# Kaz-K/medical-image-editing

Measured on AMD Instinct MI355X. Metric: images/sec (train step, 256x256 2D slices), higher is better.
Workload: dtype f32

## Files before the change

include/vqwnet_hip.h:

```cpp
#ifndef VQWNET_HIP_H
#define VQWNET_HIP_H
#include <stddef.h>
#include <stdint.h>

#define VQW_ABI_VERSION 9

#ifdef __cplusplus
extern "C" {
#endif

const char* vqw_last_error(void);
int vqw_abi_version(void);
int vqw_set_conv_backend(int mode);
int vqw_profile_begin(void);
int vqw_profile_end(double* out);
int vqw_profile_families(unsigned mask);

int vqw_conv2d_fwd(const float* src0, int C0, int up0, const float* src1, int C1,
                   const float* w_ohwi, const float* bias, float* y,
                   int N, int H, int W, int Cout, int ksize, int dil, int relu, void* stream);
int vqw_pack_dgrad_weights(const float* w_ohwi, float* wt, int Cout, int Cin, int ksize, void* stream);
int vqw_conv2d_fwd_stats_parts(int C0, int C1, int up0, int N, int H, int W, int Cout, int ksize, int dil);
int vqw_conv2d_fwd_stats(const float* src0, int C0, int up0, const float* src1, int C1,
                         const float* w_ohwi, const float* bias, float* y, float* part,
// ... 23 lines not shown
                              void* stream);
int vqw_conv3x3_up2_wgrad_supported(int Cin, int Cout, int N, int h, int w);
size_t vqw_conv3x3_up2_wgrad_ws_bytes(int Cin, int Cout, int N, int h, int w);
int vqw_conv3x3_up2_wgrad(const float* x_low, const float* dy, float* dw_ohwi, float* dbias, void* ws, size_t ws_bytes,
                          int N, int h, int w, int Cin, int Cout, int accumulate, void* stream);
int vqw_conv3x3_wino_supported(int Cin, int Cout, int N, int H, int W);
size_t vqw_conv3x3_wino_ws_bytes(int Cin, int Cout);
int vqw_conv3x3_wino_prepare(const float* w_ohwi, void* ws, size_t ws_bytes, int Cin, int Cout, void* stream);
int vqw_conv3x3_wino_prepare_dgrad(const float* w_ohwi, void* ws, size_t ws_bytes, int Cin, int Cout, void* stream);
int vqw_conv3x3_wino_fwd(const float* x, const void* ws, const float* bias, float* y, int N, int H, int W, int Cin, int Cout,
                         int relu, void* stream);
int vqw_conv3x3_wino_masked_supported(int Cin, int Cout, int N, int H, int W);
int vqw_conv3x3_wino_fwd_masked(const float* x, const void* ws, const float* mask, float* y, int N, int H, int W, int Cin,
                                int Cout, void* stream);
int vqw_conv3x3_wino_fwd_acc(const float* x, const void* ws, float* y, int N, int H, int W, int Cin, int Cout, void* stream);
int vqw_conv3x3_wino_dil2_supported(int Cin, int Cout, int N, int H, int W);
int vqw_conv3x3_wino_dil2_stats_parts(int Cin, int Cout, int N, int H, int W);
int vqw_conv3x3_wino_dil2_fwd(const float* x, const void* ws, const float* bias, float* y, float* part, int accumulate,
                              int N, int H, int W, int Cin, int Cout, int relu, void* stream);
int vqw_conv3x3_wino_split_supported(int Cin, int Cout, int split, int pool0, int N, int H, int W);
int vqw_conv3x3_wino_fwd_split(const float* x, const void* ws, const float* bias, float* y0, float* y1, int N, int H, int W,
                               int Cin, int Cout, int split, int pool0, int relu, void* stream);
int vqw_conv3x3_wino_split_padded_supported(int Cin, int Cout, int split, int c1, int pool0, int N, int H, int W);
int vqw_conv3x3_wino_fwd_split_padded(const float* x, const void* ws, const float* bias, float* y0, float* y1, int N, int H, int W,
                                      int Cin, int Cout, int split, int c1, int pool0, int relu, void* stream);
int vqw_conv3x3_wino_fwd_inbwd_parts(int Cin, int Cout, int N, int H, int W);
int vqw_conv3x3_wino_fwd_inbwd(const float* x, const void* ws, const float* norm_x, const float* norm_mean_rstd, int norm_relu,
                               float* y, float* part, int N, int H, int W, int Cin, int Cout, void* stream);
int vqw_conv3x3_wino_fwd_stats_parts(int Cin, int Cout, int N, int H, int W);
int vqw_conv3x3_wino_fwd_stats(const float* x, const void* ws, const float* bias, float* y, float* part, int N, int H, int W,
// ... 35 lines not shown
int vqw_spade_fwd(const float* x, const float* mean_rstd , const float* gamma,
                  const float* beta, int gb_stride, float* y, long P, int C, int relu, void* stream);
int vqw_spade_fwd_res(const float* x, const float* mean_rstd, const float* gamma, const float* beta, int gb_stride,
                      const float* res, float* y, long P, int C, int relu, void* stream);
int vqw_spade_fwd_res_norm_supported(long HW, int C);
int vqw_spade_fwd_res_norm(const float* x, const float* mean_rstd, const float* gamma, const float* beta, int gb_stride,
                           const float* res_raw, const float* res_mean_rstd, int res_relu, float* y, int N, long HW, int C,
                           int relu, void* stream);
int vqw_spade_bwd_reduce(const float* x, const float* mean_rstd, const float* gamma, const float* beta,
                         const float* gy, float* dgamma, float* dbeta, int gb_stride,
                         double* sums , void* ws, size_t ws_bytes, int N, int HW, int C,
                         int relu, void* stream);
int vqw_spade_bwd_apply(const float* x, const float* mean_rstd, const float* gamma, const float* beta,
                        int gb_stride, const float* gy, const double* sums, double count, float* gx,
                        long P, int C, int relu, int training, void* stream);

int vqw_add(const float* a, const float* b, float* y, long n, int relu, void* stream);
int vqw_relu_bwd(const float* y, const float* gy, float* gx, long n, void* stream);
int vqw_maxpool2_fwd(const float* x, float* y, int N, int H, int W, int C, void* stream);
int vqw_maxpool2_bwd(const float* x, const float* gy, const float* g_skip , float* gx,
                     int N, int H, int W, int C, void* stream);
int vqw_res_tail_fwd(const float* a, const float* b, float* out, float* pooled, int N, int H, int W, int C, void* stream);
int vqw_res_tail_norm_fwd(const float* x2, const float* mr2, const float* xid, const float* mrid, float* out, float* pooled,
                          int N, int H, int W, int C, void* stream);
int vqw_res_tail_bwd(const float* out, const float* g_pooled , const float* g_out , float* gx,
                     int N, int H, int W, int C, void* stream);
int vqw_tanh_fwd(const float* x, float* y, long n, void* stream);
int vqw_tanh_bwd(const float* y, const float* gy, float* gx, long n, void* stream);
int vqw_affine(const float* x, float* y, float scale, float shift, long n, void* stream);
int vqw_mse_fwd(const float* a, const float* b, float* loss, void* ws, size_t ws_bytes, long n, void* stream);
// ... 308 lines not shown
```

medical-image-editing_amd/csrc/conv.hip:

```cpp
#include "common.h"
#include <stdlib.h>
#include "conv_common.h"
#include "prof.h"
#include "../../include/vqwnet_hip.h"

static int g_conv_backend = 0;

#define PROF_MAX 32768
static bool g_prof_on = false;
static int g_prof_n = 0;
static hipEvent_t* g_prof_ev = nullptr;
static double g_prof_flops[PROF_MAX];
static double g_prof_bytes[PROF_MAX];
static int g_prof_family[PROF_MAX];

extern "C" int vqw_profile_begin(void) {
    if (!g_prof_ev) {
        g_prof_ev = (hipEvent_t*)malloc(sizeof(hipEvent_t) * 2 * PROF_MAX);
        for (int i = 0; i < 2 * PROF_MAX; ++i)
            if (hipEventCreate(&g_prof_ev[i]) != hipSuccess) { vqw_set_error("vqw_profile_begin: hipEventCreate failed"); return VQW_ERR_HIP; }
    }
    g_prof_n = 0;
    g_prof_on = true;
    return VQW_OK;
// ... 344 lines not shown
extern "C" int vqw_conv3x3_wino_fwd_masked(const float* x, const void* ws, const float* mask, float* y, int N, int H, int W, int Cin,
                                           int Cout, void* stream) {
    VQW_CHECK(x && ws && mask && y && N > 0 && H > 0 && W > 0, "vqw_conv3x3_wino_fwd_masked: bad arguments");
    VQW_CHECK(vqw_conv3x3_wino_masked_supported(Cin, Cout, N, H, W), "vqw_conv3x3_wino_fwd_masked: unsupported shape (query vqw_conv3x3_wino_masked_supported)");
    const double px = (double)N * H * W;
    ProfScope ps(4, 2.0 * px * 4.0 * Cout * Cin, (hipStream_t)stream, 4.0 * (px * Cin + 2.0 * px * Cout + 16.0 * Cout * Cin));
    return conv_wino_fwd(x, (const float*)ws, nullptr, y, N, H, W, Cin, Cout, 0, (hipStream_t)stream, nullptr, mask);
}
extern "C" int vqw_conv3x3_wino_fwd_acc(const float* x, const void* ws, float* y, int N, int H, int W, int Cin, int Cout, void* stream) {
    VQW_CHECK(x && ws && y && N > 0 && H > 0 && W > 0, "vqw_conv3x3_wino_fwd_acc: bad arguments");
    VQW_CHECK(vqw_conv3x3_wino_masked_supported(Cin, Cout, N, H, W), "vqw_conv3x3_wino_fwd_acc: unsupported shape (query vqw_conv3x3_wino_masked_supported)");
    const double px = (double)N * H * W;
    ProfScope ps(4, 2.0 * px * 4.0 * Cout * Cin, (hipStream_t)stream, 4.0 * (px * Cin + 2.0 * px * Cout + 16.0 * Cout * Cin));
    return conv_wino_fwd(x, (const float*)ws, nullptr, y, N, H, W, Cin, Cout, 0, (hipStream_t)stream, nullptr, nullptr, 1);
}
extern "C" int vqw_conv3x3_wino_dil2_supported(int Cin, int Cout, int N, int H, int W) {
    if (g_conv_backend != 0 || N < 1 || H < 2 || W < 2) return 0;
    if (!conv_wino_ok(Cin, Cout, N, H / 2, W / 2) || !conv_wino64_dil2_ok(Cin, Cout, H, W)) return 0;
    return (long)N * H * W * (Cin > Cout ? Cin : Cout) * 4 <= 0xFFFFFFE0L ? 1 : 0;
}
extern "C" int vqw_conv3x3_wino_dil2_stats_parts(int Cin, int Cout, int N, int H, int W) {
    if (!vqw_conv3x3_wino_dil2_supported(Cin, Cout, N, H, W)) return 0;
    return 4 * conv_wino64_stat_tiles(Cin, Cout, H / 2, W / 2);
}
extern "C" int vqw_conv3x3_wino_dil2_fwd(const float* x, const void* ws, const float* bias, float* y, float* part, int accumulate,
                                         int N, int H, int W, int Cin, int Cout, int relu, void* stream) {
    VQW_CHECK(x && ws && y && N > 0 && H > 0 && W > 0, "vqw_conv3x3_wino_dil2_fwd: bad arguments");
    VQW_CHECK(vqw_conv3x3_wino_dil2_supported(Cin, Cout, N, H, W), "vqw_conv3x3_wino_dil2_fwd: unsupported shape (query vqw_conv3x3_wino_dil2_supported)");
    VQW_CHECK(!part || (!relu && !accumulate && vqw_conv3x3_wino_dil2_stats_parts(Cin, Cout, N, H, W) > 0),
              "vqw_conv3x3_wino_dil2_fwd: statistics partials need relu == 0, accumulate == 0 and a served height");
// ... 73 lines not shown
```

medical-image-editing_amd/csrc/conv_common.h:

```cpp
#pragma once
#include "common.h"
#include <cstdlib>

inline int conv_max_blocks() {
    static const int v = [] {
        const char* e = getenv("VQW_CONV_MAX_BLOCKS");
        const int b = e ? atoi(e) : 256;
        return b < 8 ? 8 : (b > 256 ? 256 : b);
    }();
    return v;
}

inline int conv_slab_split(int nsp, int nblk, int max_slabs, int* kt_out) {
    int nsb = conv_max_blocks() / nblk;
    if (nsb > max_slabs) nsb = max_slabs;
    if (nsb > nsp) nsb = nsp;
    if (nsb < 1) nsb = 1;
    const int kt = (nsp + nsb - 1) / nsb;
    if (kt_out) *kt_out = kt;
    return (nsp + kt - 1) / kt;
}
inline int conv_region_runs(int nsp, int ntn, int wg_per_cu) {
    int groups = conv_max_blocks() * wg_per_cu / ntn;
    if (groups < 1) groups = 1;
// ... 77 lines not shown
bool conv_dil_wgrad_ok(const ConvIn& in, int N, int H, int W, int Cout, int ks, int dil);
int conv_dil_wgrad(const ConvIn& in, const float* dy, float* dw, float* ws, int max_slabs, int N, int H, int W, int Cout, int dil,
                   int acc, hipStream_t st);
extern int g_wino_mode;
bool conv_wino_ok(int Cin, int Cout, int N, int H, int W);
size_t conv_wino_ws_floats(int Cin, int Cout);
int conv_wino_prepare(const float* w, float* u, int Cin, int Cout, hipStream_t st, int transposed = 0);
int conv_wino_stat_tiles(int Cin, int Cout, int H, int W);
bool conv_wino64_ok(int Cin, int Cout, int W);
int conv_wino64_stat_tiles(int Cin, int Cout, int H, int W);
bool conv_wino64_split_ok(int Cin, int Cout, int split, int pool0, int N, int H, int W, int c1 = 0);
int conv_wino64_fwd_split(const float* x, const float* u, const float* bias, float* y0, float* y1, int N, int H, int W, int Cin, int Cout,
                          int split, int pool0, int relu, hipStream_t st, int c1 = 0);
int conv_wino64_fwd(const float* x, const float* u, const float* bias, float* y, int N, int H, int W, int Cin, int Cout, int relu,
                    hipStream_t st, float* stats = nullptr, const float* mask = nullptr, int accumulate = 0,
                    const float* in_mr = nullptr, int in_relu = 0, int dil = 1);
bool conv_wino64_dil2_ok(int Cin, int Cout, int H, int W);
int conv_wino_fwd(const float* x, const float* u, const float* bias, float* y, int N, int H, int W, int Cin, int Cout, int relu,
                  hipStream_t st, float* stats = nullptr, const float* mask = nullptr, int accumulate = 0,
                  const float* in_mr = nullptr, int in_relu = 0);
bool conv_wino_wgrad_ok(int Cin, int Cout, int N, int H, int W);
int conv_wino_wgrad_blocks(const ConvIn& in, int Cout, int N, int H, int W, int max_slabs, int* kt_out);
bool conv_wino_blk_wgrad_ok(int C0, int C1, int up0, int Cout, int H, int W);
bool conv_wino_blk_wgrad_dil2_ok(int C0, int Cout, int H, int W);
int conv_wino_blk_wgrad_blocks(int Cin, int Cout, int N, int H, int W, int max_slabs, int* kt_out);
int conv_wino_blk_wgrad(const ConvIn& in, const float* dy, float* ws, float* bpart, int N, int H, int W, int Cin, int Cout, int nsb, int kt,
                        hipStream_t st, int dil = 1);
int conv_wino_wgrad(const ConvIn& in, const float* dy, float* ws, float* bpart, int N, int H, int W, int Cout, int nsb, int kt,
                    hipStream_t st);
bool conv_wino_up_dgrad_ok(int Cin, int Cout, int N, int h, int w);
size_t conv_wino_up_ws_floats(int Cin, int Cout);
// ... 76 lines not shown
```

medical-image-editing_amd/csrc/conv_wino64.hip:

```cpp
#include "common.h"
#include "conv_common.h"
#include "mfma_util.h"
#include "wino_common.h"

extern int g_wino_mode;

namespace {

struct W64Args {
    const float* x;
    const float* u;
    const float* bias;
    float* y;
    int N, H, W, Cin, Cout;
    int tilesY, tilesX, nsp;
    int ntn, nch;
    int kt;
    int relu;
    unsigned nbx, nbu, nby;
    float* stats;
    const float* mask;
    const float* mr;
    int in_relu;
    float* y2;
    int split, pool0;
    int c1;
    unsigned nby2;
    unsigned img_px, rowb_px, rpx, ppx;
    int n_sh, n_m;
};

constexpr int W6_KPH = wino::KPH;
template <int RW, int MBW, int NW = 8> struct W64Geo {
    static_assert(MBW == 1 || (MBW == 2 && RW == 32), "two M blocks per wave: 32-wide regions only");
    static_assert(NW == 8 || (NW == 4 && RW == 32), "four-wave workgroups: 32-wide regions only");
    static constexpr int NMB = NW / 2;
    static constexpr int NBW = 4 / MBW;
    static constexpr int NCO = 16 * NBW;
    static constexpr int TR = RW == 32 ? 2 * MBW * NMB : 16;
    static constexpr int HR = TR + 2, HWV = RW + 2;
    static constexpr int HWS = RW == 32 ? 34 : 24;
    static constexpr int HBUF = HR * HWS * W6_KPH;
    static constexpr int UBUF = 16 * NCO * 8;
    static constexpr int EXF = 2048 * NW;
    static_assert(EXF >= UBUF, "U buffer 1 lives in the exchange area");
    static constexpr size_t LDS_FLOATS = 2 * HBUF + UBUF + EXF + 2 * NMB * NCO * 2;
};
constexpr int W6_LS = 4;
constexpr int W6_ULS = 2;
constexpr int W6_CP = 48;

template <int RW, int MBW, int EPI, int NW = 8>
__global__ void __launch_bounds__(64 * NW, 8 / NW) k_conv_wino64(W64Args a) {
    constexpr bool MASK = EPI >= 1 && EPI <= 3;
    using G = W64Geo<RW, MBW, NW>;
    constexpr int NT = 64 * NW, NMB = G::NMB, NBW = G::NBW, NCO = G::NCO;
    constexpr int HWS = G::HWS, HWV = G::HWV, HBUF = G::HBUF, UBUF = G::UBUF;
    using Halo = wino::HaloStager<NT, G::HR, HWV, HWS, wino::PitchedPix>;
    constexpr int LH = Halo::LH;
    constexpr int LU = 512 * NBW / NT;
    constexpr int HP0 = 1 + LU * W6_ULS;
    static_assert(HP0 + (LH - 1) * W6_LS < W6_CP && W6_CP + LH <= 64, "prefetch slots fit the item");

    extern __shared__ __attribute__((aligned(16))) float smem[];
    float* Hs = smem;
    float* Us = smem + 2 * HBUF;
    float* Ex = Us + UBUF;
    float* Rs = Ex + G::EXF;

    const int tid = threadIdx.x, lane = tid & 63;
    const int wv = __builtin_amdgcn_readfirstlane(tid >> 6);
    const int mb = wv & (NMB - 1), h = wv / NMB;
    const int H = a.H, W = a.W, Cin = a.Cin, Cout = a.Cout;
    const __amdgpu_buffer_rsrc_t rsx = make_rsrc(a.x, a.nbx), rsu = make_rsrc(a.u, a.nbu), rsy = make_rsrc(a.y, a.nby);
    const __amdgpu_buffer_rsrc_t rsm = make_rsrc((EPI == 1 || EPI == 3) ? a.mask : a.y, a.nby);
    const __amdgpu_buffer_rsrc_t rsr = make_rsrc(EPI == 3 ? a.mr : a.y, EPI == 3 ? (unsigned)((size_t)a.N * a.Cout * 8) : a.nby);
    const __amdgpu_buffer_rsrc_t rsy2 = make_rsrc(EPI == 4 ? a.y2 : a.y, EPI == 4 ? a.nby2 : a.nby);

    const int nch = a.nch;
    const wino::RegionRun run = wino::region_run(a.ntn, a.kt, a.nsp);
    const int co_base = run.tile_n * NCO;
    const int my_tiles = run.my_tiles;
    if (my_tiles <= 0) return;

    const int c4 = tid & 1;
    const wino::PitchedPix pixel = {a.img_px, a.rowb_px, a.rpx, a.ppx, a.n_sh, a.n_m};
    Halo hs;
    hs.init(tid, pixel);
    auto region_offsets = [&](int n, int tx, int ty) { hs.region_offsets(n, ty * G::TR - 1, tx * RW - 1, H, W, Cin); };
    const int u_n = (tid >> 1) & (NCO - 1);
    const int u_swz = (u_n >> 3) & 1;
    const int u_c4 = c4 ^ u_swz;
    const unsigned u_voff = (((unsigned)(tid >> 1) / NCO * Cout + co_base + u_n) * 8u + u_c4 * 4) * 4u;
    const unsigned u_jstride = (unsigned)(NT / 2 / NCO) * Cout * 32u;
    const unsigned u_cstride = 16u * Cout * 32u;
    const int u_wave = wv * 256;

    auto issue_h = [&](int j, int chunk) { hs.issue_h(rsx, j, chunk); };
    auto commit_h = [&](int j, float* Hb) { hs.commit_h(j, Hb); };
    auto issue_u = [&](int j, int chunk, float* Ub) {
        wino::buf_ld4_lds(rsu, Ub + u_wave + j * (NT * 4), u_voff, chunk * u_cstride + j * u_jstride);
    };

    int cn, ctx, cty, ch = 0;
    region_start(run.sp0, a.tilesY, a.tilesX, cn, ctx, cty);
    auto advance = [&](int& n, int& tx, int& ty, int& c) {
        const int adv = c + 1 == nch ? 1 : 0;
        c = adv ? 0 : c + 1;
        region_step(adv, a.tilesY, a.tilesX, n, tx, ty);
    };
    int n1 = cn, tx1 = ctx, ty1 = cty, ch1 = 0;
    advance(n1, tx1, ty1, ch1);
    int n2 = n1, tx2 = tx1, ty2 = ty1, ch2 = ch1;
// ... 340 lines not shown
}

static int wino64_shape(int Cin, int Cout, int W) {
    if (Cin % 16 != 0) return 0;
    if (Cout % 64 == 0) return 1;
    return (Cout % 32 == 0 && W % 32 == 0) ? 2 : 0;
}
static int wino64_waves(int shape) { return shape == 2 ? 4 : 8; }
bool conv_wino64_ok(int Cin, int Cout, int W) { return wino64_shape(Cin, Cout, W) != 0; }
int conv_wino64_stat_tiles(int Cin, int Cout, int H, int W) {
    const int shape = wino64_shape(Cin, Cout, W);
    const int rw = W % 32 == 0 ? 32 : 16, tr = rw == 32 ? shape * wino64_waves(shape) : 16;
    return tr > 0 && H % tr == 0 ? (H / tr) * (W / rw) : 0;
}

template <int RW, int MBW, int EPI, int NW = 8>
static int launch_wino64(W64Args& a, hipStream_t st) {
    using G = W64Geo<RW, MBW, NW>;
    constexpr size_t lds = G::LDS_FLOATS * sizeof(float);
    static_assert(lds * (8 / NW) <= 160 * 1024, "buffers do not fit the 160 KB LDS");
    if (int rc = lds_opt_in<k_conv_wino64<RW, MBW, EPI, NW>>((int)lds, "conv_wino64")) return rc;
    a.tilesY = ceil_div(a.H, G::TR); a.tilesX = a.W / RW; a.nsp = a.N * a.tilesY * a.tilesX;
    a.ntn = a.Cout / G::NCO;
    a.kt = conv_region_runs(a.nsp, a.ntn, 8 / NW);
    k_conv_wino64<RW, MBW, EPI, NW><<<ceil_div(a.nsp, a.kt) * a.ntn, 64 * NW, lds, st>>>(a);
    VQW_LAUNCH_CHECK("conv_wino64");
    return VQW_OK;
}

bool conv_wino64_dil2_ok(int Cin, int Cout, int H, int W) {
    return H % 2 == 0 && W % 64 == 0 && wino64_shape(Cin, Cout, W / 2) != 0;
}
int conv_wino64_fwd(const float* x, const float* u, const float* bias, float* y, int N, int H, int W, int Cin, int Cout, int relu,
                    hipStream_t st, float* stats, const float* mask, int accumulate, const float* in_mr, int in_relu, int dil) {
    W64Args a;
    const long P = (long)N * H * W;
    a.img_px = (unsigned)(H * W); a.rowb_px = 0; a.rpx = (unsigned)W; a.ppx = 1; a.n_sh = 0; a.n_m = 0;
    if (dil == 2) {
        a.rowb_px = (unsigned)W; a.rpx = 2u * (unsigned)W; a.ppx = 2; a.n_sh = 2; a.n_m = 1;
        N *= 4; H /= 2; W /= 2;
    }
    a.y2 = nullptr; a.split = 0; a.pool0 = 0; a.c1 = 0; a.nby2 = 0;
    a.x = x; a.u = u; a.bias = bias; a.y = y; a.mask = mask; a.mr = in_mr; a.in_relu = in_relu;
    a.N = N; a.H = H; a.W = W; a.Cin = Cin; a.Cout = Cout;
    a.nch = Cin / 8;
    a.relu = relu;
    a.stats = stats;
    a.nbx = (unsigned)(P * Cin * 4);
    a.nbu = (unsigned)(16L * Cout * Cin * 4);
    a.nby = (unsigned)(P * Cout * 4);
    const int shape = wino64_shape(Cin, Cout, W);
    if (in_mr) {
        if (shape == 2) return launch_wino64<32, 2, 3, 4>(a, st);
        if (W % 32 == 0) return launch_wino64<32, 1, 3>(a, st);
        return launch_wino64<16, 1, 3>(a, st);
    }
    if (mask) {
        if (shape == 2) return launch_wino64<32, 2, 1, 4>(a, st);
        if (W % 32 == 0) return launch_wino64<32, 1, 1>(a, st);
        return launch_wino64<16, 1, 1>(a, st);
    }
    if (accumulate) {
        if (shape == 2) return launch_wino64<32, 2, 2, 4>(a, st);
        if (W % 32 == 0) return launch_wino64<32, 1, 2>(a, st);
        return launch_wino64<16, 1, 2>(a, st);
    }
    if (shape == 2) return launch_wino64<32, 2, 0, 4>(a, st);
    if (W % 32 == 0) return launch_wino64<32, 1, 0>(a, st);
    return launch_wino64<16, 1, 0>(a, st);
}

bool conv_wino64_split_ok(int Cin, int Cout, int split, int pool0, int N, int H, int W, int c1) {
    if (c1 < 0 || c1 % 16 != 0 || split + c1 > Cout) return false;
    if (!conv_wino64_ok(Cin, Cout, W) || g_wino_mode != 0 || split <= 0 || split >= Cout || split % 16 != 0) return false;
    if (pool0 && (H % 2 != 0)) return false;
    return (long)N * H * W * (Cin > Cout ? Cin : Cout) * 4 <= 0xFFFFFFE0L;
}
int conv_wino64_fwd_split(const float* x, const float* u, const float* bias, float* y0, float* y1, int N, int H, int W, int Cin, int Cout,
                          int split, int pool0, int relu, hipStream_t st, int c1) {
    if (c1 <= 0) c1 = Cout - split;
    W64Args a;
    a.img_px = (unsigned)(H * W); a.rowb_px = 0; a.rpx = (unsigned)W; a.ppx = 1; a.n_sh = 0; a.n_m = 0;
    a.x = x; a.u = u; a.bias = bias; a.y = y0; a.y2 = y1; a.mask = nullptr; a.mr = nullptr; a.in_relu = 0;
    a.split = split; a.pool0 = pool0; a.c1 = c1;
    a.N = N; a.H = H; a.W = W; a.Cin = Cin; a.Cout = Cout;
    a.nch = Cin / 8;
    a.relu = relu;
    a.stats = nullptr;
    const long P = (long)N * H * W;
    a.nbx = (unsigned)(P * Cin * 4);
    a.nbu = (unsigned)(16L * Cout * Cin * 4);
    a.nby = (unsigned)((pool0 ? P / 4 : P) * split * 4);
    a.nby2 = (unsigned)(P * c1 * 4);
    const int shape = wino64_shape(Cin, Cout, W);
    if (shape == 2) return launch_wino64<32, 2, 4, 4>(a, st);
    if (W % 32 == 0) return launch_wino64<32, 1, 4>(a, st);
    return launch_wino64<16, 1, 4>(a, st);
}
// ... 357 lines not shown
```

medical-image-editing_amd/csrc/norm.hip:

```cpp
#include <type_traits>
#include "common.h"
#include "prof.h"
#include "../../include/vqwnet_hip.h"

#define PLANE_MAX_SPLITS 64

static inline int plane_splits(int N, int HW) {
    int s = ceil_div(2048, N);
    int cap = imax(1, HW / 256);
    s = imin(imin(s, cap), PLANE_MAX_SPLITS);
    return imax(s, 1);
}

static inline size_t plane_part_bytes(int N, int C) { return (size_t)N * PLANE_MAX_SPLITS * C * 2 * sizeof(double); }
extern "C" size_t vqw_plane_ws_bytes(int N, int C, int HW) {
    (void)HW;
    return plane_part_bytes(N, C) + (size_t)N * C * 2 * sizeof(float);
}

__device__ __forceinline__ float norm_xhat(float x, float mean, float rstd) { return (x - mean) * rstd; }
__device__ __forceinline__ void stats_terms(float v, float& a, float& b) { a = v; b = v * v; }
__device__ __forceinline__ float inorm_bwd_term(float g, float xh, bool relu) { return (relu && !(xh > 0.f)) ? 0.f : g; }
__device__ __forceinline__ float inorm_bwd_out(float gg, float xh, float rstd, float e0, float e1) { return rstd * (gg - e0 - xh * e1); }
__device__ __forceinline__ float spade_out(float xh, float gamma, float beta) { return xh * (1.f + gamma) + beta; }
// ... 770 lines not shown
            }
#pragma unroll
        for (int u = 0; u < 4; ++u) {
            if (p0 + u * R >= P) break;
            float4 o = spade4(v[u], ga[u], be[u], m0, m1, RELU);
            if (RES) { o.x += rr[u].x; o.y += rr[u].y; o.z += rr[u].z; o.w += rr[u].w; }
            y[(p0 + u * R) * C4 + c4] = o;
        }
    }
}

template <int RELU, int TRAIN>
__global__ void __launch_bounds__(256) k_spade_bwd_apply4w(const float4* __restrict__ x, const float* __restrict__ mr,
                                                           const float4* __restrict__ gamma, const float4* __restrict__ beta,
                                                           const float4* __restrict__ gy, const double* __restrict__ sums,
                                                           double inv_count, float4* __restrict__ gx, long P, int C4, int lgC4, int gbs4) {
    WALK4_SETUP;
    const float4 m0 = ((const float4*)(mr + 8 * c4))[0], m1 = ((const float4*)(mr + 8 * c4))[1];
    float s1[4], s2[4];
    spade_bwd_means4(sums, inv_count, c4, TRAIN, s1, s2);
    for (long p0 = (long)blockIdx.x * 2 * R + r; p0 < P; p0 += (long)gridDim.x * 2 * R) {
        float4 v[2], ga4[2], g4[2], be4[2];
#pragma unroll
        for (int u = 0; u < 2; ++u)
            if (p0 + u * R < P) {
                const long p = p0 + u * R;
                v[u] = x[p * C4 + c4]; ga4[u] = gamma[p * gbs4 + c4]; g4[u] = gy[p * C4 + c4];
                be4[u] = RELU ? beta[p * gbs4 + c4] : make_float4(0.f, 0.f, 0.f, 0.f);
            }
#pragma unroll
        for (int u = 0; u < 2; ++u) {
            if (p0 + u * R >= P) break;
            gx[(p0 + u * R) * C4 + c4] = spade_bwd4(v[u], g4[u], ga4[u], be4[u], m0, m1, s1, s2, RELU, TRAIN);
        }
    }
}
static inline int walk_blocks_flat(long P, int C4, int per_step) {
    const int R = 256 / C4;
    long g = (P + (long)per_step * R - 1) / ((long)per_step * R);
    return (int)(g > 2048 ? 2048 : (g < 1 ? 1 : g));
}

// ... 527 lines not shown
    with_flag(relu, [&](auto R) {
        constexpr int RELU = decltype(R)::value;
        if (pick_tier(C, gb_stride, x, gamma, beta, gy, dgamma, dbeta, mean_rstd) != TIER_SCALAR)
            splits = launch_plane_reduce4(FSpadeBwd4<RELU>{(const float4*)x, mean_rstd, (const float4*)gamma, (const float4*)beta, (const float4*)gy,
                                                           (float4*)dgamma, (float4*)dbeta, C / 4, gb_stride / 4}, (double*)ws, N, HW, C, st);
        else splits = launch_plane_reduce(FSpadeBwd<RELU>{x, mean_rstd, gamma, beta, gy, dgamma, dbeta, C, gb_stride}, (double*)ws, N, HW, C, st);
    });
    k_channel_finalize<SplitSums, false><<<C, 256, 0, st>>>(SplitSums{(const double*)ws, N * splits}, sums, C, BnOut{});
    VQW_LAUNCH_CHECK("vqw_spade_bwd_reduce");
    return VQW_OK;
}

template <int RELU, int TRAIN>
__global__ void k_spade_bwd_apply(const float* __restrict__ x, const float* __restrict__ mr, const float* __restrict__ gamma,
                                  const float* __restrict__ beta, const float* __restrict__ gy, const double* __restrict__ sums,
                                  double inv_count, float* __restrict__ gx, long total, int C, int gbs) {
    long stride = (long)gridDim.x * blockDim.x;
    for (long i = (long)blockIdx.x * blockDim.x + threadIdx.x; i < total; i += stride) {
        int c = (int)(i % C);
        long j = (i / C) * gbs + c;
        float r = mr[2 * c + 1];
        float xh = norm_xhat(x[i], mr[2 * c], r);
        float dg, db, dxh;
        spade_bwd_grad(gy[i], xh, gamma[j], RELU ? beta[j] : 0.f, RELU, dg, db, dxh);
        float s1 = TRAIN ? (float)(sums[2 * c] * inv_count) : 0.f;
        float s2 = TRAIN ? (float)(sums[2 * c + 1] * inv_count) : 0.f;
        gx[i] = spade_bwd_out(dxh, xh, r, s1, s2, TRAIN);
    }
}
template <int RELU, int TRAIN>
__global__ void __launch_bounds__(256) k_spade_bwd_apply4(const float4* __restrict__ x, const float* __restrict__ mr,
                                                          const float4* __restrict__ gamma, const float4* __restrict__ beta,
                                                          const float4* __restrict__ gy, const double* __restrict__ sums,
                                                          double inv_count, float4* __restrict__ gx, long total4, int C4, int gbs4) {
    long stride = (long)gridDim.x * blockDim.x;
    for (long i = (long)blockIdx.x * blockDim.x + threadIdx.x; i < total4; i += stride) {
        int c4 = (int)(i % C4);
        long j = (i / C4) * gbs4 + c4;
        const float4* m = (const float4*)(mr + 8 * c4);
        const float4 m0 = m[0], m1 = m[1], v = x[i], ga = gamma[j], g = gy[i];
        const float4 be = RELU ? beta[j] : make_float4(0.f, 0.f, 0.f, 0.f);
        float s1[4], s2[4];
        spade_bwd_means4(sums, inv_count, c4, TRAIN, s1, s2);
        gx[i] = spade_bwd4(v, g, ga, be, m0, m1, s1, s2, RELU, TRAIN);
    }
}
extern "C" int vqw_spade_bwd_apply(const float* x, const float* mean_rstd, const float* gamma, const float* beta, int gb_stride,
                                   const float* gy, const double* sums, double count, float* gx, long P, int C,
                                   int relu, int training, void* stream) {
    VQW_PROF_HBM(stream, 4, (double)P * C);
    VQW_CHECK(x && mean_rstd && gamma && beta && gy && gx && P > 0 && C > 0 && gb_stride >= C, "vqw_spade_bwd_apply: bad arguments");
    VQW_CHECK(!training || (sums && count > 0), "vqw_spade_bwd_apply: training needs sums and count");
    const long total = P * C;
    hipStream_t st = (hipStream_t)stream;
    const double ic = training ? 1.0 / count : 0.0;
    const Tier tier = pick_tier(C, gb_stride, x, gamma, beta, gy, gx, mean_rstd);
    const int C4 = C / 4, s4 = gb_stride / 4;
    const float4 *x4 = (const float4*)x, *ga4 = (const float4*)gamma, *be4 = (const float4*)beta, *gy4 = (const float4*)gy;
    with_flag(relu, [&](auto R) {
        with_flag(training, [&](auto T) {
            constexpr int RELU = decltype(R)::value, TRAIN = decltype(T)::value;
            if (tier == TIER_WALK4)
                k_spade_bwd_apply4w<RELU, TRAIN><<<walk_blocks_flat(P, C4, 2), 256, 0, st>>>(x4, mean_rstd, ga4, be4, gy4, sums, ic, (float4*)gx, P, C4, ilog2_exact(C4), s4);
            else if (tier == TIER_FLAT4)
                k_spade_bwd_apply4<RELU, TRAIN><<<stream_grid(total / 4, 256), 256, 0, st>>>(x4, mean_rstd, ga4, be4, gy4, sums, ic, (float4*)gx, total / 4, C4, s4);
            else k_spade_bwd_apply<RELU, TRAIN><<<stream_grid(total, 256), 256, 0, st>>>(x, mean_rstd, gamma, beta, gy, sums, ic, gx, total, C, gb_stride);
        });
    });
    VQW_LAUNCH_CHECK("vqw_spade_bwd_apply");
    return VQW_OK;
}

__global__ void k_bn_affine_fwd(const float* __restrict__ x, const float* __restrict__ mr, const float* __restrict__ gamma,
                                const float* __restrict__ beta, float* __restrict__ y, long total, int C, float slope) {
    long stride = (long)gridDim.x * blockDim.x;
    for (long i = (long)blockIdx.x * blockDim.x + threadIdx.x; i < total; i += stride) {
        int c = (int)(i % C);
        float v = ((x[i] - mr[2 * c]) * mr[2 * c + 1]) * gamma[c] + beta[c];
        y[i] = v > 0.f ? v : v * slope;
    }
}
extern "C" int vqw_bn_affine_fwd(const float* x, const float* mean_rstd, const float* gamma, const float* beta, float* y, long P,
                                 int C, float slope, void* stream) {
    VQW_CHECK(x && mean_rstd && gamma && beta && y && P > 0 && C > 0, "vqw_bn_affine_fwd: bad arguments");
// ... 70 lines not shown
```

medical-image-editing_amd/hipops/ops.py:

```python
import contextlib
import ctypes
import math
import os

import torch
import torch.distributed as dist

from . import _lib
from .library import Dispatch as _D

CL = torch.channels_last


_dispatch = None


def _L():
    global _dispatch
    if _dispatch is None:
        _dispatch = _D()
    return _dispatch


def _raw(t):
# ... 467 lines not shown
        self._armed_for = None

    def put(self, grad, payload):
        tid = _pass_id()
        if tid >= 0 and self._armed_for != tid:
            self._armed_for = tid
            torch.autograd.Variable._execution_engine.queue_callback(self.clear)
        self.notes[grad.data_ptr()] = (grad._version, tid, payload)

    def take(self, grad):
        ent = self.notes.pop(grad.data_ptr(), None)
        if ent is None or ent[0] != grad._version or ent[1] != _pass_id():
            return None
        return ent[2]

    def clear(self):
        self.notes.clear()
        self._armed_for = None

    def __len__(self):
        return len(self.notes)


UP_PAIR = os.environ.get("VQW_UP_PAIR", "1") != "0"
up_pair_calls = 0
CONV_PAIR = os.environ.get("VQW_CONV_PAIR", "1") != "0"
conv_pair_calls = 0


class _ConvPair(torch.autograd.Function):

    @staticmethod
    def forward(ctx, x, wa, ba, wb, bb, relu, group, up):
        global up_pair_calls, conv_pair_calls
        _dev(x, wa, ba, wb, bb)
        x = nhwc(x)
        Ca, Cin, ks, _ = wa.shape
        N, _, h, w = x.shape
        L = _L()
        deps = (wb,) + tuple(t for t in (ba, bb) if t is not None)
        if up:
            nparts = L.vqw_conv3x3_up2_fwd_pair_supported(Cin, Ca, N, h, w)
# ... 29 lines not shown
        ctx.cfg = (N, H, W, Ca, Cin)
        ctx.params = ((wa, ba), (wb, bb))
        ctx.defer = [_out_of_band(ctx.needs_input_grad[1 + 2 * i], params, w_n is params[0])
                     for i, (params, w_n) in enumerate(zip(ctx.params, (wa_n, wb_n)))]
        ctx.set_materialize_grads(False)
        return outs

    @staticmethod
    def backward(ctx, *grads):
        x, wa_n, wb_n, ya, yb = ctx.saved_tensors
        N, H, W, Cout, Cin = ctx.cfg
        up = ctx.up
        L = _L()
        out = [None] * 8
        gx_total = None
        for i in (1, 0):
            gy = grads[2 * i] if up else grads[i]
            if gy is None:
                if ctx.group is not None:
                    raise RuntimeError("%s: both outputs must take part in the backward pass of a gradient group"
                                       % ("conv2d_up_pair" if up else "conv2d_pair"))
                continue
            wgt, bias = ctx.params[i]
            w_n = (wa_n, wb_n)[i]
            up_ws = _cached(wgt, "up2", lambda: _up2_weights(L, w_n, Cin, Cout)) if up else None
            need0 = ctx.needs_input_grad[0]
            needw, needb = ctx.needs_input_grad[1 + 2 * i], (bias is not None and ctx.needs_input_grad[2 + 2 * i])
            defer = ctx.defer[i] and (needw or needb)
            g0, _, gw, gbias, gy_n = conv2d_backward_impl(gy, x, None, w_n, (ya, yb)[i], 1, up, bias is not None, up_ws, need0, False,
                                                          needw and not defer, needb and not defer, group=ctx.group)
            if defer:
                _deferred_wgrad(wgt, bias if (bias is not None and bias.requires_grad) else None, x, None, gy_n, up, 3, 1,
                                N, H, W, Cout, collapsed=up)
            out[1 + 2 * i], out[2 + 2 * i] = gw, gbias
            if g0 is not None:
                gx_total = g0 if gx_total is None else gx_total.add_(g0)
        out[0] = gx_total
        return tuple(out)


def conv2d_up_pair_supported(x, weight_a, weight_b):
    if not (UP_PAIR and x.is_cuda and weight_a.shape == weight_b.shape and weight_a.shape[2] == 3 and not _in_custom_op):
        return False
    N, _, h, w = x.shape
    return _L().vqw_conv3x3_up2_fwd_pair_supported(weight_a.shape[1], weight_a.shape[0], N, h, w) > 0


def conv2d_up_pair(x, weight_a, bias_a, weight_b, bias_b, grad_group=None):
    ya, pa, yb, pb = _ConvPair.apply(x, weight_a, bias_a, weight_b, bias_b, False, grad_group if GRAD_GROUPS else None, True)
    return (ya, pa), (yb, pb)


def conv2d_pair_supported(x, weight_a, weight_b):
# ... 507 lines not shown
        gy = nhwc(gy)
        if fused:
            dgamma, dbeta, gbs = torch.empty_like(gamma, memory_format=CL), None, 2 * C
            gptr, dgptr = gamma, dgamma
            bptr, dbptr = gamma.narrow(1, C, C), dgamma.narrow(1, C, C)
        else:
            dgamma = torch.empty_like(x, memory_format=CL)
            dbeta = torch.empty_like(x, memory_format=CL)
            gbs, gptr, bptr, dgptr, dbptr = C, gamma, beta, dgamma, dbeta
        gx = torch.empty_like(x, memory_format=CL)
        sums = torch.empty(2 * C, dtype=torch.float64, device=x.device)
        ws = _ws(L.vqw_plane_ws_bytes(N, C, H * W), x)
        L.vqw_spade_bwd_reduce(x, mr, gptr, bptr, gy, dgptr, dbptr, gbs, sums, ws, ws.numel(), N, H * W, C, int(relu))
        if training and sync and _dist_on():
            _all_reduce(sums)
        L.vqw_spade_bwd_apply(x, mr, gptr, bptr, gbs, gy, sums, count, gx, N * H * W, C, int(relu), int(training))
        gres = gy if ctx.has_res else None
        if rmr is not None and ctx.needs_input_grad[11]:
            gres = _inorm_bwd(res_raw, rmr, gy, ctx.res_relu)
        return gx, dgamma, dbeta, None, None, None, None, None, None, None, None, gres, None, None


RES_NORM_FUSED = os.environ.get("VQW_RES_NORM_FUSED", "1") != "0"


def spade_norm(x, gamma, beta, running_mean, running_var, training, momentum=0.1, eps=1e-5, relu=False, sync=True,
               num_batches_tracked=None, residual=None, part=None, residual_norm=None):
    if residual is not None and residual_norm is not None:
        N, C, H, W = x.shape
        if not (RES_NORM_FUSED and x.is_cuda and not (C & 3) and not (gamma.shape[1] & 3) and tuple(residual.shape) == tuple(x.shape)
                and _L().vqw_spade_fwd_res_norm_supported(H * W, C)):
            rpart, rrelu, reps = residual_norm
            residual = instance_norm(residual, relu=rrelu, eps=reps, part=rpart)
            residual_norm = None
    if residual_norm is not None:
        return _Spade.apply(x, gamma, beta, running_mean, running_var, bool(training), float(momentum), float(eps), bool(relu),
                            bool(sync), num_batches_tracked, residual, part if training else None,
# ... 2865 lines not shown
```

Baseline: 361.7.

## Fuse paired conv dgrad into one two-source Winograd launch and reuse dbeta in SPADE apply

Adds a two-source Winograd forward kernel variant that reads the two output gradients of a conv pair from separate buffers. The pair's input gradient is then computed with one launch over concatenated flipped weights, replacing two dgrads plus an add. SPADE backward apply now reads the already-masked gradient (dbeta) instead of recomputing from gy and beta, which saves reads and the relu branch. Both paths add cached weight transforms and rely on correct masked-grad bookkeeping.

```diff
diff --git a/include/vqwnet_hip.h b/include/vqwnet_hip.h
--- a/include/vqwnet_hip.h
+++ b/include/vqwnet_hip.h
@@ -61,6 +61,9 @@
 int vqw_conv3x3_wino_fwd_masked(const float* x, const void* ws, const float* mask, float* y, int N, int H, int W, int Cin,
                                 int Cout, void* stream);
 int vqw_conv3x3_wino_fwd_acc(const float* x, const void* ws, float* y, int N, int H, int W, int Cin, int Cout, void* stream);
+int vqw_conv3x3_wino_fwd2_supported(int Cs, int Cout, int N, int H, int W);
+int vqw_conv3x3_wino_fwd2(const float* x0, const float* x1, const void* ws, float* y, int accumulate, int N, int H, int W, int Cs,
+                          int Cout, void* stream);
 int vqw_conv3x3_wino_dil2_supported(int Cin, int Cout, int N, int H, int W);
 int vqw_conv3x3_wino_dil2_stats_parts(int Cin, int Cout, int N, int H, int W);
 int vqw_conv3x3_wino_dil2_fwd(const float* x, const void* ws, const float* bias, float* y, float* part, int accumulate,
@@ -126,6 +129,9 @@
 int vqw_spade_bwd_apply(const float* x, const float* mean_rstd, const float* gamma, const float* beta,
                         int gb_stride, const float* gy, const double* sums, double count, float* gx,
                         long P, int C, int relu, int training, void* stream);
+int vqw_spade_bwd_apply_gm(const float* x, const float* mean_rstd, const float* gamma, int gamma_stride, const float* gm,
+                           int gm_stride, const double* sums, double count, float* gx, long P, int C, int training,
+                           void* stream);
 
 int vqw_add(const float* a, const float* b, float* y, long n, int relu, void* stream);
 int vqw_relu_bwd(const float* y, const float* gy, float* gx, long n, void* stream);
diff --git a/medical-image-editing_amd/csrc/conv.hip b/medical-image-editing_amd/csrc/conv.hip
--- a/medical-image-editing_amd/csrc/conv.hip
+++ b/medical-image-editing_amd/csrc/conv.hip
@@ -382,6 +382,19 @@
     ProfScope ps(4, 2.0 * px * 4.0 * Cout * Cin, (hipStream_t)stream, 4.0 * (px * Cin + 2.0 * px * Cout + 16.0 * Cout * Cin));
     return conv_wino_fwd(x, (const float*)ws, nullptr, y, N, H, W, Cin, Cout, 0, (hipStream_t)stream, nullptr, nullptr, 1);
 }
+extern "C" int vqw_conv3x3_wino_fwd2_supported(int Cs, int Cout, int N, int H, int W) {
+    if (g_conv_backend != 0 || Cs < 8 || !conv_wino_ok(2 * Cs, Cout, N, H, W) || !conv_wino64_two_ok(Cs, Cout, W)) return 0;
+    return (long)N * H * W * (Cs > Cout ? Cs : Cout) * 4 <= 0xFFFFFFE0L ? 1 : 0;
+}
+extern "C" int vqw_conv3x3_wino_fwd2(const float* x0, const float* x1, const void* ws, float* y, int accumulate, int N, int H, int W,
+                                     int Cs, int Cout, void* stream) {
+    VQW_CHECK(x0 && x1 && ws && y && N > 0 && H > 0 && W > 0, "vqw_conv3x3_wino_fwd2: bad arguments");
+    VQW_CHECK(vqw_conv3x3_wino_fwd2_supported(Cs, Cout, N, H, W), "vqw_conv3x3_wino_fwd2: unsupported shape (query vqw_conv3x3_wino_fwd2_supported)");
+    const double px = (double)N * H * W;
+    ProfScope ps(4, 2.0 * px * 4.0 * Cout * 2.0 * Cs, (hipStream_t)stream, 4.0 * (px * 2.0 * Cs + (accumulate ? 2.0 : 1.0) * px * Cout + 32.0 * Cout * Cs));
+    return conv_wino64_fwd(x0, (const float*)ws, nullptr, y, N, H, W, 2 * Cs, Cout, 0, (hipStream_t)stream, nullptr, nullptr, accumulate ? 1 : 0,
+                           nullptr, 0, 1, x1);
+}
 extern "C" int vqw_conv3x3_wino_dil2_supported(int Cin, int Cout, int N, int H, int W) {
     if (g_conv_backend != 0 || N < 1 || H < 2 || W < 2) return 0;
     if (!conv_wino_ok(Cin, Cout, N, H / 2, W / 2) || !conv_wino64_dil2_ok(Cin, Cout, H, W)) return 0;
diff --git a/medical-image-editing_amd/csrc/conv_common.h b/medical-image-editing_amd/csrc/conv_common.h
--- a/medical-image-editing_amd/csrc/conv_common.h
+++ b/medical-image-editing_amd/csrc/conv_common.h
@@ -115,7 +115,8 @@
                           int split, int pool0, int relu, hipStream_t st, int c1 = 0);
 int conv_wino64_fwd(const float* x, const float* u, const float* bias, float* y, int N, int H, int W, int Cin, int Cout, int relu,
                     hipStream_t st, float* stats = nullptr, const float* mask = nullptr, int accumulate = 0,
-                    const float* in_mr = nullptr, int in_relu = 0, int dil = 1);
+                    const float* in_mr = nullptr, int in_relu = 0, int dil = 1, const float* x1 = nullptr);
+bool conv_wino64_two_ok(int Cs, int Cout, int W);
 bool conv_wino64_dil2_ok(int Cin, int Cout, int H, int W);
 int conv_wino_fwd(const float* x, const float* u, const float* bias, float* y, int N, int H, int W, int Cin, int Cout, int relu,
                   hipStream_t st, float* stats = nullptr, const float* mask = nullptr, int accumulate = 0,
diff --git a/medical-image-editing_amd/csrc/conv_wino64.hip b/medical-image-editing_amd/csrc/conv_wino64.hip
--- a/medical-image-editing_amd/csrc/conv_wino64.hip
+++ b/medical-image-editing_amd/csrc/conv_wino64.hip
@@ -28,6 +28,8 @@
     unsigned nby2;
     unsigned img_px, rowb_px, rpx, ppx;
     int n_sh, n_m;
+    const float* x1;
+    int nch0, cpx;
 };
 
 constexpr int W6_KPH = wino::KPH;
@@ -50,7 +52,7 @@
 constexpr int W6_ULS = 2;
 constexpr int W6_CP = 48;
 
-template <int RW, int MBW, int EPI, int NW = 8>
+template <int RW, int MBW, int EPI, int NW = 8, bool TWO = false>
 __global__ void __launch_bounds__(64 * NW, 8 / NW) k_conv_wino64(W64Args a) {
     constexpr bool MASK = EPI >= 1 && EPI <= 3;
     using G = W64Geo<RW, MBW, NW>;
@@ -72,7 +74,7 @@
     const int wv = __builtin_amdgcn_readfirstlane(tid >> 6);
     const int mb = wv & (NMB - 1), h = wv / NMB;
     const int H = a.H, W = a.W, Cin = a.Cin, Cout = a.Cout;
-    const __amdgpu_buffer_rsrc_t rsx = make_rsrc(a.x, a.nbx), rsu = make_rsrc(a.u, a.nbu), rsy = make_rsrc(a.y, a.nby);
+    const __amdgpu_buffer_rsrc_t rsx = make_rsrc(a.x, a.nbx), rsx1 = make_rsrc(TWO ? a.x1 : a.x, a.nbx), rsu = make_rsrc(a.u, a.nbu), rsy = make_rsrc(a.y, a.nby);
     const __amdgpu_buffer_rsrc_t rsm = make_rsrc((EPI == 1 || EPI == 3) ? a.mask : a.y, a.nby);
     const __amdgpu_buffer_rsrc_t rsr = make_rsrc(EPI == 3 ? a.mr : a.y, EPI == 3 ? (unsigned)((size_t)a.N * a.Cout * 8) : a.nby);
     const __amdgpu_buffer_rsrc_t rsy2 = make_rsrc(EPI == 4 ? a.y2 : a.y, EPI == 4 ? a.nby2 : a.nby);
@@ -87,7 +89,7 @@
     const wino::PitchedPix pixel = {a.img_px, a.rowb_px, a.rpx, a.ppx, a.n_sh, a.n_m};
     Halo hs;
     hs.init(tid, pixel);
-    auto region_offsets = [&](int n, int tx, int ty) { hs.region_offsets(n, ty * G::TR - 1, tx * RW - 1, H, W, Cin); };
+    auto region_offsets = [&](int n, int tx, int ty) { hs.region_offsets(n, ty * G::TR - 1, tx * RW - 1, H, W, TWO ? a.cpx : Cin); };
     const int u_n = (tid >> 1) & (NCO - 1);
     const int u_swz = (u_n >> 3) & 1;
     const int u_c4 = c4 ^ u_swz;
@@ -96,7 +98,12 @@
     const unsigned u_cstride = 16u * Cout * 32u;
     const int u_wave = wv * 256;
 
-    auto issue_h = [&](int j, int chunk) { hs.issue_h(rsx, j, chunk); };
+    auto issue_h = [&](int j, int chunk) {
+        if (TWO) {
+            const bool src1 = chunk >= a.nch0;
+            hs.issue_h(src1 ? rsx1 : rsx, j, chunk - (src1 ? a.nch0 : 0));
+        } else hs.issue_h(rsx, j, chunk);
+    };
     auto commit_h = [&](int j, float* Hb) { hs.commit_h(j, Hb); };
     auto issue_u = [&](int j, int chunk, float* Ub) {
         wino::buf_ld4_lds(rsu, Ub + u_wave + j * (NT * 4), u_voff, chunk * u_cstride + j * u_jstride);
@@ -467,27 +474,30 @@
     return tr > 0 && H % tr == 0 ? (H / tr) * (W / rw) : 0;
 }
 
-template <int RW, int MBW, int EPI, int NW = 8>
+template <int RW, int MBW, int EPI, int NW = 8, bool TWO = false>
 static int launch_wino64(W64Args& a, hipStream_t st) {
     using G = W64Geo<RW, MBW, NW>;
     constexpr size_t lds = G::LDS_FLOATS * sizeof(float);
     static_assert(lds * (8 / NW) <= 160 * 1024, "buffers do not fit the 160 KB LDS");
-    if (int rc = lds_opt_in<k_conv_wino64<RW, MBW, EPI, NW>>((int)lds, "conv_wino64")) return rc;
+    if (int rc = lds_opt_in<k_conv_wino64<RW, MBW, EPI, NW, TWO>>((int)lds, "conv_wino64")) return rc;
     a.tilesY = ceil_div(a.H, G::TR); a.tilesX = a.W / RW; a.nsp = a.N * a.tilesY * a.tilesX;
     a.ntn = a.Cout / G::NCO;
     a.kt = conv_region_runs(a.nsp, a.ntn, 8 / NW);
-    k_conv_wino64<RW, MBW, EPI, NW><<<ceil_div(a.nsp, a.kt) * a.ntn, 64 * NW, lds, st>>>(a);
+    k_conv_wino64<RW, MBW, EPI, NW, TWO><<<ceil_div(a.nsp, a.kt) * a.ntn, 64 * NW, lds, st>>>(a);
     VQW_LAUNCH_CHECK("conv_wino64");
     return VQW_OK;
 }
 
+bool conv_wino64_two_ok(int Cs, int Cout, int W) { return Cs > 0 && Cs % 8 == 0 && wino64_shape(2 * Cs, Cout, W) != 0; }
 bool conv_wino64_dil2_ok(int Cin, int Cout, int H, int W) {
     return H % 2 == 0 && W % 64 == 0 && wino64_shape(Cin, Cout, W / 2) != 0;
 }
 int conv_wino64_fwd(const float* x, const float* u, const float* bias, float* y, int N, int H, int W, int Cin, int Cout, int relu,
-                    hipStream_t st, float* stats, const float* mask, int accumulate, const float* in_mr, int in_relu, int dil) {
+                    hipStream_t st, float* stats, const float* mask, int accumulate, const float* in_mr, int in_relu, int dil,
+                    const float* x1) {
     W64Args a;
     const long P = (long)N * H * W;
+    a.x1 = x1 ? x1 : x; a.cpx = x1 ? Cin / 2 : Cin; a.nch0 = x1 ? Cin / 16 : Cin / 8;
     a.img_px = (unsigned)(H * W); a.rowb_px = 0; a.rpx = (unsigned)W; a.ppx = 1; a.n_sh = 0; a.n_m = 0;
     if (dil == 2) {
         a.rowb_px = (unsigned)W; a.rpx = 2u * (unsigned)W; a.ppx = 2; a.n_sh = 2; a.n_m = 1;
@@ -499,7 +509,7 @@
     a.nch = Cin / 8;
     a.relu = relu;
     a.stats = stats;
-    a.nbx = (unsigned)(P * Cin * 4);
+    a.nbx = (unsigned)(P * a.cpx * 4);
     a.nbu = (unsigned)(16L * Cout * Cin * 4);
     a.nby = (unsigned)(P * Cout * 4);
     const int shape = wino64_shape(Cin, Cout, W);
@@ -513,6 +523,16 @@
         if (W % 32 == 0) return launch_wino64<32, 1, 1>(a, st);
         return launch_wino64<16, 1, 1>(a, st);
     }
+    if (x1) {
+        if (accumulate) {
+            if (shape == 2) return launch_wino64<32, 2, 2, 4, true>(a, st);
+            if (W % 32 == 0) return launch_wino64<32, 1, 2, 8, true>(a, st);
+            return launch_wino64<16, 1, 2, 8, true>(a, st);
+        }
+        if (shape == 2) return launch_wino64<32, 2, 0, 4, true>(a, st);
+        if (W % 32 == 0) return launch_wino64<32, 1, 0, 8, true>(a, st);
+        return launch_wino64<16, 1, 0, 8, true>(a, st);
+    }
     if (accumulate) {
         if (shape == 2) return launch_wino64<32, 2, 2, 4>(a, st);
         if (W % 32 == 0) return launch_wino64<32, 1, 2>(a, st);
@@ -535,6 +555,7 @@
     W64Args a;
     a.img_px = (unsigned)(H * W); a.rowb_px = 0; a.rpx = (unsigned)W; a.ppx = 1; a.n_sh = 0; a.n_m = 0;
     a.x = x; a.u = u; a.bias = bias; a.y = y0; a.y2 = y1; a.mask = nullptr; a.mr = nullptr; a.in_relu = 0;
+    a.x1 = x; a.cpx = Cin; a.nch0 = Cin / 8;
     a.split = split; a.pool0 = pool0; a.c1 = c1;
     a.N = N; a.H = H; a.W = W; a.Cin = Cin; a.Cout = Cout;
     a.nch = Cin / 8;
diff --git a/medical-image-editing_amd/csrc/norm.hip b/medical-image-editing_amd/csrc/norm.hip
--- a/medical-image-editing_amd/csrc/norm.hip
+++ b/medical-image-editing_amd/csrc/norm.hip
@@ -808,7 +808,8 @@
 __global__ void __launch_bounds__(256) k_spade_bwd_apply4w(const float4* __restrict__ x, const float* __restrict__ mr,
                                                            const float4* __restrict__ gamma, const float4* __restrict__ beta,
                                                            const float4* __restrict__ gy, const double* __restrict__ sums,
-                                                           double inv_count, float4* __restrict__ gx, long P, int C4, int lgC4, int gbs4) {
+                                                           double inv_count, float4* __restrict__ gx, long P, int C4, int lgC4, int gbs4,
+                                                           int gys4) {
     WALK4_SETUP;
     const float4 m0 = ((const float4*)(mr + 8 * c4))[0], m1 = ((const float4*)(mr + 8 * c4))[1];
     float s1[4], s2[4];
@@ -819,7 +820,7 @@
         for (int u = 0; u < 2; ++u)
             if (p0 + u * R < P) {
                 const long p = p0 + u * R;
-                v[u] = x[p * C4 + c4]; ga4[u] = gamma[p * gbs4 + c4]; g4[u] = gy[p * C4 + c4];
+                v[u] = x[p * C4 + c4]; ga4[u] = gamma[p * gbs4 + c4]; g4[u] = gy[p * gys4 + c4];
                 be4[u] = RELU ? beta[p * gbs4 + c4] : make_float4(0.f, 0.f, 0.f, 0.f);
             }
 #pragma unroll
@@ -1377,7 +1378,7 @@
 template <int RELU, int TRAIN>
 __global__ void k_spade_bwd_apply(const float* __restrict__ x, const float* __restrict__ mr, const float* __restrict__ gamma,
                                   const float* __restrict__ beta, const float* __restrict__ gy, const double* __restrict__ sums,
-                                  double inv_count, float* __restrict__ gx, long total, int C, int gbs) {
+                                  double inv_count, float* __restrict__ gx, long total, int C, int gbs, int gys) {
     long stride = (long)gridDim.x * blockDim.x;
     for (long i = (long)blockIdx.x * blockDim.x + threadIdx.x; i < total; i += stride) {
         int c = (int)(i % C);
@@ -1385,7 +1386,7 @@
         float r = mr[2 * c + 1];
         float xh = norm_xhat(x[i], mr[2 * c], r);
         float dg, db, dxh;
-        spade_bwd_grad(gy[i], xh, gamma[j], RELU ? beta[j] : 0.f, RELU, dg, db, dxh);
+        spade_bwd_grad(gy[(i / C) * gys + c], xh, gamma[j], RELU ? beta[j] : 0.f, RELU, dg, db, dxh);
         float s1 = TRAIN ? (float)(sums[2 * c] * inv_count) : 0.f;
         float s2 = TRAIN ? (float)(sums[2 * c + 1] * inv_count) : 0.f;
         gx[i] = spade_bwd_out(dxh, xh, r, s1, s2, TRAIN);
@@ -1395,18 +1396,39 @@
 __global__ void __launch_bounds__(256) k_spade_bwd_apply4(const float4* __restrict__ x, const float* __restrict__ mr,
                                                           const float4* __restrict__ gamma, const float4* __restrict__ beta,
                                                           const float4* __restrict__ gy, const double* __restrict__ sums,
-                                                          double inv_count, float4* __restrict__ gx, long total4, int C4, int gbs4) {
+                                                          double inv_count, float4* __restrict__ gx, long total4, int C4, int gbs4,
+                                                          int gys4) {
     long stride = (long)gridDim.x * blockDim.x;
     for (long i = (long)blockIdx.x * blockDim.x + threadIdx.x; i < total4; i += stride) {
         int c4 = (int)(i % C4);
         long j = (i / C4) * gbs4 + c4;
         const float4* m = (const float4*)(mr + 8 * c4);
-        const float4 m0 = m[0], m1 = m[1], v = x[i], ga = gamma[j], g = gy[i];
+        const float4 m0 = m[0], m1 = m[1], v = x[i], ga = gamma[j], g = gy[(i / C4) * gys4 + c4];
         const float4 be = RELU ? beta[j] : make_float4(0.f, 0.f, 0.f, 0.f);
         float s1[4], s2[4];
         spade_bwd_means4(sums, inv_count, c4, TRAIN, s1, s2);
         gx[i] = spade_bwd4(v, g, ga, be, m0, m1, s1, s2, RELU, TRAIN);
     }
+}
+static int launch_spade_bwd_apply(const float* x, const float* mean_rstd, const float* gamma, const float* beta, int gb_stride,
+                                  const float* gy, int gy_stride, const double* sums, double count, float* gx, long P, int C, int relu,
+                                  int training, hipStream_t st) {
+    const long total = P * C;
+    const double ic = training ? 1.0 / count : 0.0;
+    const Tier tier = pick_tier(C, gb_stride | gy_stride, x, gamma, beta, gy, gx, mean_rstd);
+    const int C4 = C / 4, s4 = gb_stride / 4, g4 = gy_stride / 4;
+    const float4 *x4 = (const float4*)x, *ga4 = (const float4*)gamma, *be4 = (const float4*)beta, *gy4 = (const float4*)gy;
+    with_flag(relu, [&](auto R) {
+        with_flag(training, [&](auto T) {
+            constexpr int RELU = decltype(R)::value, TRAIN = decltype(T)::value;
+            if (tier == TIER_WALK4)
+                k_spade_bwd_apply4w<RELU, TRAIN><<<walk_blocks_flat(P, C4, 2), 256, 0, st>>>(x4, mean_rstd, ga4, be4, gy4, sums, ic, (float4*)gx, P, C4, ilog2_exact(C4), s4, g4);
+            else if (tier == TIER_FLAT4)
+                k_spade_bwd_apply4<RELU, TRAIN><<<stream_grid(total / 4, 256), 256, 0, st>>>(x4, mean_rstd, ga4, be4, gy4, sums, ic, (float4*)gx, total / 4, C4, s4, g4);
+            else k_spade_bwd_apply<RELU, TRAIN><<<stream_grid(total, 256), 256, 0, st>>>(x, mean_rstd, gamma, beta, gy, sums, ic, gx, total, C, gb_stride, gy_stride);
+        });
+    });
+    return VQW_OK;
 }
 extern "C" int vqw_spade_bwd_apply(const float* x, const float* mean_rstd, const float* gamma, const float* beta, int gb_stride,
                                    const float* gy, const double* sums, double count, float* gx, long P, int C,
@@ -1414,23 +1436,18 @@
     VQW_PROF_HBM(stream, 4, (double)P * C);
     VQW_CHECK(x && mean_rstd && gamma && beta && gy && gx && P > 0 && C > 0 && gb_stride >= C, "vqw_spade_bwd_apply: bad arguments");
     VQW_CHECK(!training || (sums && count > 0), "vqw_spade_bwd_apply: training needs sums and count");
-    const long total = P * C;
-    hipStream_t st = (hipStream_t)stream;
-    const double ic = training ? 1.0 / count : 0.0;
-    const Tier tier = pick_tier(C, gb_stride, x, gamma, beta, gy, gx, mean_rstd);
-    const int C4 = C / 4, s4 = gb_stride / 4;
-    const float4 *x4 = (const float4*)x, *ga4 = (const float4*)gamma, *be4 = (const float4*)beta, *gy4 = (const float4*)gy;
-    with_flag(relu, [&](auto R) {
-        with_flag(training, [&](auto T) {
-            constexpr int RELU = decltype(R)::value, TRAIN = decltype(T)::value;
-            if (tier == TIER_WALK4)
-                k_spade_bwd_apply4w<RELU, TRAIN><<<walk_blocks_flat(P, C4, 2), 256, 0, st>>>(x4, mean_rstd, ga4, be4, gy4, sums, ic, (float4*)gx, P, C4, ilog2_exact(C4), s4);
-            else if (tier == TIER_FLAT4)
-                k_spade_bwd_apply4<RELU, TRAIN><<<stream_grid(total / 4, 256), 256, 0, st>>>(x4, mean_rstd, ga4, be4, gy4, sums, ic, (float4*)gx, total / 4, C4, s4);
-            else k_spade_bwd_apply<RELU, TRAIN><<<stream_grid(total, 256), 256, 0, st>>>(x, mean_rstd, gamma, beta, gy, sums, ic, gx, total, C, gb_stride);
-        });
-    });
+    launch_spade_bwd_apply(x, mean_rstd, gamma, beta, gb_stride, gy, C, sums, count, gx, P, C, relu, training, (hipStream_t)stream);
     VQW_LAUNCH_CHECK("vqw_spade_bwd_apply");
+    return VQW_OK;
+}
+extern "C" int vqw_spade_bwd_apply_gm(const float* x, const float* mean_rstd, const float* gamma, int gamma_stride, const float* gm,
+                                      int gm_stride, const double* sums, double count, float* gx, long P, int C, int training,
+                                      void* stream) {
+    VQW_PROF_HBM(stream, 4, (double)P * C);
+    VQW_CHECK(x && mean_rstd && gamma && gm && gx && P > 0 && C > 0 && gamma_stride >= C && gm_stride >= C, "vqw_spade_bwd_apply_gm: bad arguments");
+    VQW_CHECK(!training || (sums && count > 0), "vqw_spade_bwd_apply_gm: training needs sums and count");
+    launch_spade_bwd_apply(x, mean_rstd, gamma, gamma, gamma_stride, gm, gm_stride, sums, count, gx, P, C, 0, training, (hipStream_t)stream);
+    VQW_LAUNCH_CHECK("vqw_spade_bwd_apply_gm");
     return VQW_OK;
 }
 
diff --git a/medical-image-editing_amd/hipops/ops.py b/medical-image-editing_amd/hipops/ops.py
--- a/medical-image-editing_amd/hipops/ops.py
+++ b/medical-image-editing_amd/hipops/ops.py
@@ -505,6 +505,12 @@
             return None
         return ent[2]
 
+    def peek(self, grad):
+        ent = self.notes.get(grad.data_ptr())
+        if ent is None or ent[0] != grad._version or ent[1] != _pass_id():
+            return None
+        return ent[2]
+
     def clear(self):
         self.notes.clear()
         self._armed_for = None
@@ -517,6 +523,8 @@
 up_pair_calls = 0
 CONV_PAIR = os.environ.get("VQW_CONV_PAIR", "1") != "0"
 conv_pair_calls = 0
+PAIR_DGRAD = os.environ.get("VQW_PAIR_DGRAD", "1") != "0"
+pair_dgrad_calls = 0
 
 
 class _ConvPair(torch.autograd.Function):
@@ -576,7 +584,24 @@
         L = _L()
         out = [None] * 8
         gx_total = None
+        fused = not up and _ConvPair._fused_dgrad(ctx, grads, x, wa_n, wb_n, ya, yb)
+        if fused:
+            out[0] = fused[0]
         for i in (1, 0):
+            if fused:
+                wgt, bias = ctx.params[i]
+                needw, needb = ctx.needs_input_grad[1 + 2 * i], (bias is not None and ctx.needs_input_grad[2 + 2 * i])
+                defer = ctx.defer[i] and (needw or needb)
+                gy_n = fused[1][i]
+                if defer:
+                    _deferred_wgrad(wgt, bias if (bias is not None and bias.requires_grad) else None, x, None, gy_n, False, 3, 1,
+                                    N, H, W, Cout)
+                elif needw or needb:
+                    gw = torch.empty((Cout, Cin, 3, 3), dtype=torch.float32, device=gy_n.device, memory_format=CL)
+                    gbias = torch.empty(Cout, dtype=torch.float32, device=gy_n.device) if bias is not None else None
+                    _run_wgrad(L, x, None, gy_n, gw, gbias, False, 3, 1, N, H, W, Cout, False, False)
+                    out[1 + 2 * i], out[2 + 2 * i] = (gw if needw else None), (gbias if needb else None)
+                continue
             gy = grads[2 * i] if up else grads[i]
             if gy is None:
                 if ctx.group is not None:
@@ -597,8 +622,38 @@
             out[1 + 2 * i], out[2 + 2 * i] = gw, gbias
             if g0 is not None:
                 gx_total = g0 if gx_total is None else gx_total.add_(g0)
-        out[0] = gx_total
+        if not fused:
+            out[0] = gx_total
         return tuple(out)
+
+    @staticmethod
+    def _fused_dgrad(ctx, grads, x, wa_n, wb_n, ya, yb):
+        global pair_dgrad_calls
+        if not PAIR_DGRAD or not ctx.needs_input_grad[0] or grads[0] is None or grads[1] is None:
+            return None
+        N, H, W, Cout, Cin = ctx.cfg
+        L = _L()
+        group = ctx.group
+        if group is not None and not (group.members == 2 and group.remaining == 2 and group.buf is None):
+            return None
+        if not L.vqw_conv3x3_wino_fwd2_supported(Cout, Cin, N, H, W):
+            return None
+        if ya is not None and not (_MASKED_GRADS.peek(grads[0]) == ya.data_ptr() and _MASKED_GRADS.peek(grads[1]) == yb.data_ptr()):
+            return None
+        if ya is not None:
+            _MASKED_GRADS.take(grads[0])
+            _MASKED_GRADS.take(grads[1])
+        ga, gb_ = nhwc(grads[0]), nhwc(grads[1])
+        wa, wb = ctx.params[0][0], ctx.params[1][0]
+        ut = _cached(wa, "pair_wino_dgrad", lambda: _wino_weights_dgrad(L, _concat_layers(wa_n, None, wb_n, None)[0], 2 * Cout, Cin),
+                     deps=(wb,))
+        gx = torch.empty_like(x, memory_format=CL)
+        L.vqw_conv3x3_wino_fwd2(ga, gb_, ut, gx, 0, N, H, W, Cout, Cin)
+        pair_dgrad_calls += 1
+        if group is not None:
+            group.member_done(gx)
+            gx = group.member_done(None)
+        return gx, (ga, gb_)
 
 
 def conv2d_up_pair_supported(x, weight_a, weight_b):
@@ -1136,13 +1191,17 @@
         L.vqw_spade_bwd_reduce(x, mr, gptr, bptr, gy, dgptr, dbptr, gbs, sums, ws, ws.numel(), N, H * W, C, int(relu))
         if training and sync and _dist_on():
             _all_reduce(sums)
-        L.vqw_spade_bwd_apply(x, mr, gptr, bptr, gbs, gy, sums, count, gx, N * H * W, C, int(relu), int(training))
+        if SPADE_APPLY_GM:
+            L.vqw_spade_bwd_apply_gm(x, mr, gptr, gbs, dbptr, gbs, sums, count, gx, N * H * W, C, int(training))
+        else:
+            L.vqw_spade_bwd_apply(x, mr, gptr, bptr, gbs, gy, sums, count, gx, N * H * W, C, int(relu), int(training))
         gres = gy if ctx.has_res else None
         if rmr is not None and ctx.needs_input_grad[11]:
             gres = _inorm_bwd(res_raw, rmr, gy, ctx.res_relu)
         return gx, dgamma, dbeta, None, None, None, None, None, None, None, None, gres, None, None
 
 
+SPADE_APPLY_GM = os.environ.get("VQW_SPADE_APPLY_GM", "1") != "0"
 RES_NORM_FUSED = os.environ.get("VQW_RES_NORM_FUSED", "1") != "0"
 
 
```

New measurement: 364.6 (median of 6 runs). No clear change (+0.8%).
